# arclabs561/innr

Measured on NVIDIA B200. Metric: batch_knn_cosine_top10_queries_per_s, higher is better.
Workload: dtype f32

## Files before the change

### innr_b200/csrc/scan_f32.cu

```cuda
#include <algorithm>
#include <cmath>
#include <type_traits>

#include "common.cuh"
#include "kernels.cuh"
#include "pdx.cuh"

namespace innr {

namespace {

constexpr int SCAN_THREADS = 256;
constexpr int VPT = 4;
constexpr int TILE = SCAN_THREADS * VPT;
constexpr float NORM_EPS = 1e-9f;

struct PdxArgs {
  PdxView v;
  unsigned long long ld;
  unsigned n, d, ld4;
  unsigned n_tiles;
  unsigned index_base;
  const float* queries;
  int nq_valid;
// ... 726 lines not shown
    float ss = 0.0f;
    for (unsigned i = 0; i < d; ++i) ss = __fadd_rn(ss, __fmul_rn(query[i], query[i]));
    s_qn = __fsqrt_rn(ss);
  }
  __syncthreads();
  const unsigned j = blockIdx.x * blockDim.x + threadIdx.x;
  if (j >= m) return;
  const unsigned gid = cand[j];
  const unsigned i = gid - index_base;
  if (gid < index_base || i >= n) {
    out[j] = MODE == PDX_L2 ? __int_as_float(0x7FC00000) : __int_as_float(0xFFC00000);
    return;
  }
  float acc = 0.0f, ss = 0.0f;
  for (unsigned dd = 0; dd < d; ++dd) {
    const float x = pdx_load1(v, (size_t)dd * v.ld + i);
    accumulate<MODE == PDX_COSINE_FUSED ? PDX_DOT : MODE>(sq[dd], x, acc);
    if (MODE == PDX_COSINE_FUSED) ss = __fadd_rn(ss, __fmul_rn(x, x));
  }
  float sc = acc;
  if (MODE == PDX_COSINE_FUSED) {
    const float nrm = __fsqrt_rn(ss), qn = s_qn;
    sc = (!(qn < NORM_EPS) && nrm > NORM_EPS) ? __fdiv_rn(acc, __fmul_rn(qn, nrm)) : 0.0f;
  }
  out[j] = sc;
}
}

cudaError_t launch_subset_scores(const PdxView& v, int mode, const float* dev_query, const uint32_t* dev_cand, size_t m,
                                 float* dev_out, cudaStream_t s, LaunchCounter* launches) {
  if (m == 0) return cudaSuccess;
  const unsigned grid = (unsigned)((m + SCAN_THREADS - 1) / SCAN_THREADS);
  const size_t smem = ((v.d + 3) & ~(size_t)3) * sizeof(float);
  if (smem > 200 * 1024) return cudaErrorInvalidValue;
#define INNR_SUBSET(MODE)                                                                                           \
  {                                                                                                                 \
    auto kern = subset_scores_kernel<MODE>;                                                                         \
    if (smem > 48 * 1024) {                                                                                         \
      cudaError_t e = cudaFuncSetAttribute(kern, cudaFuncAttributeMaxDynamicSharedMemorySize, (int)smem);           \
      if (e != cudaSuccess) return e;                                                                               \
    }                                                                                                               \
    kern<<<grid, SCAN_THREADS, smem, s>>>(v, (unsigned)v.n, (unsigned)v.d, v.index_base, dev_query,                 \
                                          dev_cand, (unsigned)m, dev_out);                                          \
  }
  if (mode == PDX_DOT) INNR_SUBSET(PDX_DOT)
  else if (mode == PDX_L2) INNR_SUBSET(PDX_L2)
  else if (mode == PDX_COSINE_FUSED) INNR_SUBSET(PDX_COSINE_FUSED)
  else return cudaErrorInvalidValue;
#undef INNR_SUBSET
  ++*launches;
  return cudaGetLastError();
}

cudaError_t launch_topk_from_scores(const void* dev_scores, int kind, size_t n, uint32_t index_base, size_t k,
                                    uint64_t* dev_keys, Workspace& ws, cudaStream_t s, LaunchCounter* launches,
                                    const uint32_t* dev_ids, const uint32_t* dev_mask, unsigned seg_len, unsigned seg_stride) {
  unsigned grid = (unsigned)((n + SCAN_THREADS - 1) / SCAN_THREADS);
  unsigned cap = (unsigned)ws.num_sms * 4u;
  if (grid > cap) grid = cap;
  if (grid == 0) grid = 1;
  for (size_t done = 0; done < k; done += 128) {
    const int kr = (int)std::min<size_t>(128, k - done);
    const uint64_t* floor = done ? dev_keys + done - 1 : nullptr;
    uint64_t* out = dev_keys + done;
    const size_t smem = (size_t)(SCAN_THREADS / 32) * kr * sizeof(uint64_t);
#define INNR_TOPK_LAUNCH(R, KIND)                                                                                   \
  topk_scores_kernel<R, KIND><<<grid, SCAN_THREADS, smem, s>>>(dev_scores, (unsigned)n, index_base, dev_ids, dev_mask, seg_len, seg_stride, kr, floor, \
                                                               ws.partials, ws.group_partials, out, ws.tickets)
    if (kr <= 32) {
      if (kind == 0) INNR_TOPK_LAUNCH(1, 0); else if (kind == 1) INNR_TOPK_LAUNCH(1, 1);
      else if (kind == 2) INNR_TOPK_LAUNCH(1, 2); else if (kind == 3) INNR_TOPK_LAUNCH(1, 3); else INNR_TOPK_LAUNCH(1, 4);
    } else {
      if (kind == 0) INNR_TOPK_LAUNCH(4, 0); else if (kind == 1) INNR_TOPK_LAUNCH(4, 1);
      else if (kind == 2) INNR_TOPK_LAUNCH(4, 2); else if (kind == 3) INNR_TOPK_LAUNCH(4, 3); else INNR_TOPK_LAUNCH(4, 4);
    }
#undef INNR_TOPK_LAUNCH
    ++*launches;
    cudaError_t e = cudaGetLastError();
    if (e != cudaSuccess) return e;
  }
  return cudaSuccess;
}

namespace {
__global__ void decode_keys_kernel(const uint64_t* __restrict__ keys, size_t total, int descending, uint64_t* __restrict__ idx,
                                   float* __restrict__ score) {
  const size_t t = (size_t)blockIdx.x * blockDim.x + threadIdx.x;
  if (t >= total) return;
  const uint64_t key = keys[t];
  if (idx) idx[t] = key & 0xFFFFFFFFull;
  if (score) {
    uint32_t hi = (uint32_t)(key >> 32);
    if (descending) hi = ~hi;
    score[t] = __uint_as_float(order_bits_to_f32_bits(hi));
  }
}
}

cudaError_t launch_merge_keys_big(const uint64_t* dev_in, size_t n_lists, size_t nq, size_t k, int descending,
                                  uint64_t* dev_keys_out, uint64_t* dev_idx, float* dev_score, Workspace& ws, cudaStream_t s,
                                  LaunchCounter* launches) {
  for (size_t q = 0; q < nq; ++q) {
    cudaError_t e = launch_topk_from_scores(dev_in + q * k, 3, n_lists * k, 0, k, dev_keys_out + q * k, ws, s, launches, nullptr,
                                            nullptr, (unsigned)k, (unsigned)(nq * k));
    if (e != cudaSuccess) return e;
  }
  if (dev_idx || dev_score) {
    const size_t total = nq * k;
    decode_keys_kernel<<<(unsigned)((total + 255) / 256), 256, 0, s>>>(dev_keys_out, total, descending, dev_idx, dev_score);
    ++*launches;
  }
  return cudaGetLastError();
}

namespace {

struct AdaptArgs {
  PdxView v;
  unsigned long long ld;
  unsigned ld4;
  const float* query;
  unsigned d0, d1;
  float* dist;
  const uint32_t* mask_in;
  uint32_t* mask_out;
  const float* thr;
  uint32_t* ev;
  unsigned* pruned;
  int no_prune;
};

__global__ void __launch_bounds__(SCAN_THREADS) adaptive_epoch_kernel(const AdaptArgs a) {
  extern __shared__ __align__(16) unsigned char smem_raw[];
  float* sq = reinterpret_cast<float*>(smem_raw);
  const unsigned nd = a.d1 - a.d0;
  for (unsigned j = threadIdx.x; j < nd; j += blockDim.x) sq[j] = a.query[a.d0 + j];
  __syncthreads();
  const int lane = threadIdx.x & 31;
  const unsigned i0 = (blockIdx.x * SCAN_THREADS + threadIdx.x) * VPT;
  const bool in = i0 < a.ld4;
  unsigned nib = in ? (a.mask_in[i0 >> 5] >> (i0 & 31)) & 0xFu : 0u;
  unsigned n_dead = 0;
  if (nib) {
    float4 acc = *reinterpret_cast<const float4*>(a.dist + i0);
    const float T = a.thr[0];
    unsigned ex = 0, e0 = 0, e1 = 0, e2 = 0, e3 = 0;
    size_t p = (size_t)a.d0 * a.ld + i0;
    auto step = [&](const float4& v, unsigned j) {
      const float q = sq[j];
      float df;
      df = __fsub_rn(q, v.x); acc.x = __fadd_rn(acc.x, __fmul_rn(df, df));
      df = __fsub_rn(q, v.y); acc.y = __fadd_rn(acc.y, __fmul_rn(df, df));
      df = __fsub_rn(q, v.z); acc.z = __fadd_rn(acc.z, __fmul_rn(df, df));
      df = __fsub_rn(q, v.w); acc.w = __fadd_rn(acc.w, __fmul_rn(df, df));
      if (!(ex & 1u) && acc.x > T) { ex |= 1u; e0 = a.d0 + j; }
      if (!(ex & 2u) && acc.y > T) { ex |= 2u; e1 = a.d0 + j; }
      if (!(ex & 4u) && acc.z > T) { ex |= 4u; e2 = a.d0 + j; }
      if (!(ex & 8u) && acc.w > T) { ex |= 8u; e3 = a.d0 + j; }
    };
    constexpr int U = 8;
    unsigned j = 0;
    for (; j + U <= nd; j += U) {
      float4 v[U];
#pragma unroll
      for (int u = 0; u < U; ++u) v[u] = pdx_load4(a.v, p + (size_t)u * a.ld);
      p += (size_t)U * a.ld;
#pragma unroll
      for (int u = 0; u < U; ++u) step(v[u], j + u);
    }
    for (; j < nd; ++j) {
      const float4 v = pdx_load4(a.v, p);
      p += a.ld;
      step(v, j);
    }
    *reinterpret_cast<float4*>(a.dist + i0) = acc;
    if (!a.no_prune) {
      const unsigned dead = ex & nib;
      if (dead & 1u) a.ev[i0] = e0;
      if (dead & 2u) a.ev[i0 + 1] = e1;
      if (dead & 4u) a.ev[i0 + 2] = e2;
      if (dead & 8u) a.ev[i0 + 3] = e3;
      nib &= ~dead;
      n_dead = __popc(dead);
    }
  }
  unsigned w = nib << (4 * (lane & 7));
  w |= __shfl_xor_sync(FULL_MASK, w, 1);
  w |= __shfl_xor_sync(FULL_MASK, w, 2);
  w |= __shfl_xor_sync(FULL_MASK, w, 4);
  if (in && (lane & 7) == 0) a.mask_out[i0 >> 5] = w;
#pragma unroll
  for (int o = 16; o > 0; o >>= 1) n_dead += __shfl_xor_sync(FULL_MASK, n_dead, o);
  if (lane == 0 && n_dead) atomicAdd(a.pruned, n_dead);
}

__global__ void adaptive_threshold_kernel(const uint64_t* key, float scale, float* thr) {
  const float t = __fmul_rn(__uint_as_float(order_bits_to_f32_bits((uint32_t)(*key >> 32))), scale);
  thr[0] = t;
  thr[1] = __fmul_rn(t, 1.5f);
}

__global__ void __launch_bounds__(SCAN_THREADS) adaptive_mark_kernel(const float* __restrict__ dist, unsigned n, unsigned ld4,
                                                                    float ratio, const float* __restrict__ thr,
                                                                    uint32_t* __restrict__ mask_out, unsigned* pruned) {
  const int lane = threadIdx.x & 31;
  const unsigned i = blockIdx.x * SCAN_THREADS + threadIdx.x;
  const unsigned words32 = (ld4 + 31u) / 32u * 32u;
  bool alive = false, dead = false;
  if (i < n) {
    dead = __fmul_rn(dist[i], ratio) > thr[1];
    alive = !dead;
  }
  const unsigned w = __ballot_sync(FULL_MASK, alive);
  const unsigned nd = __popc(__ballot_sync(FULL_MASK, dead));
  if (lane == 0) {
    if (i < words32) mask_out[i >> 5] = w;
    if (nd) atomicAdd(pruned, nd);
  }
}

__global__ void __launch_bounds__(SCAN_THREADS) adaptive_event_keys_kernel(const uint32_t* __restrict__ before,
                                                                          const uint32_t* __restrict__ after,
                                                                          const uint32_t* __restrict__ ev, unsigned n,
                                                                          uint64_t* __restrict__ keys) {
  const unsigned i = blockIdx.x * SCAN_THREADS + threadIdx.x;
  if (i >= n) return;
  const bool event = ((before[i >> 5] & ~after[i >> 5]) >> (i & 31)) & 1u;
  keys[i] = event ? ~(((uint64_t)ev[i] << 32) | i) : KEY_SENTINEL;
}

__global__ void adaptive_revive_kernel(const uint64_t* __restrict__ keys, unsigned m, uint32_t* mask) {
  const unsigned t = blockIdx.x * blockDim.x + threadIdx.x;
  if (t >= m) return;
  const unsigned i = (unsigned)(~keys[t] & 0xFFFFFFFFull);
  atomicOr(mask + (i >> 5), 1u << (i & 31));
}

}

cudaError_t launch_adaptive_threshold(const uint64_t* dev_key, float scale, float* dev_thr, cudaStream_t s,
                                      LaunchCounter* launches) {
  adaptive_threshold_kernel<<<1, 1, 0, s>>>(dev_key, scale, dev_thr);
  ++*launches;
  return cudaGetLastError();
}

cudaError_t launch_adaptive_mark(const PdxView& v, const float* dev_dist, float ratio, const float* dev_thr,
                                 uint32_t* dev_mask_out, unsigned* dev_pruned, cudaStream_t s, LaunchCounter* launches) {
  const unsigned ld4 = (unsigned)std::min<size_t>(v.ld, (v.n + 3) / 4 * 4);
  const unsigned span = (ld4 + 31u) / 32u * 32u;
  adaptive_mark_kernel<<<(span + SCAN_THREADS - 1) / SCAN_THREADS, SCAN_THREADS, 0, s>>>(dev_dist, (unsigned)v.n, ld4, ratio,
                                                                                      dev_thr, dev_mask_out, dev_pruned);
  ++*launches;
  return cudaGetLastError();
}

cudaError_t launch_adaptive_epoch(const PdxView& v, const float* dev_query, size_t d0, size_t d1, float* dev_dist,
                                  const uint32_t* dev_mask_in, uint32_t* dev_mask_out, const float* dev_thr, uint32_t* dev_ev,
                                  unsigned* dev_pruned, int no_prune, cudaStream_t s, LaunchCounter* launches) {
  AdaptArgs a{};
  a.v = v;
  a.ld = v.ld;
  a.ld4 = (unsigned)std::min<size_t>(v.ld, (v.n + 3) / 4 * 4);
  a.query = dev_query;
  a.d0 = (unsigned)d0;
  a.d1 = (unsigned)d1;
  a.dist = dev_dist;
  a.mask_in = dev_mask_in;
  a.mask_out = dev_mask_out;
  a.thr = dev_thr;
  a.ev = dev_ev;
  a.pruned = dev_pruned;
  a.no_prune = no_prune;
  const unsigned span = (a.ld4 + 31u) / 32u * 32u;
  const unsigned grid = (span / VPT + SCAN_THREADS - 1) / SCAN_THREADS;
  adaptive_epoch_kernel<<<grid, SCAN_THREADS, (d1 - d0) * sizeof(float), s>>>(a);
  ++*launches;
  return cudaGetLastError();
}

cudaError_t launch_adaptive_event_keys(const uint32_t* dev_before, const uint32_t* dev_after, const uint32_t* dev_ev, size_t n,
                                       uint64_t* dev_keys, cudaStream_t s, LaunchCounter* launches) {
  adaptive_event_keys_kernel<<<(unsigned)((n + SCAN_THREADS - 1) / SCAN_THREADS), SCAN_THREADS, 0, s>>>(dev_before, dev_after,
                                                                                                     dev_ev, (unsigned)n, dev_keys);
  ++*launches;
  return cudaGetLastError();
}

cudaError_t launch_adaptive_revive(const uint64_t* dev_keys, size_t m, uint32_t* dev_mask, cudaStream_t s,
                                   LaunchCounter* launches) {
  if (m == 0) return cudaSuccess;
  adaptive_revive_kernel<<<(unsigned)((m + 255) / 256), 256, 0, s>>>(dev_keys, (unsigned)m, dev_mask);
  ++*launches;
  return cudaGetLastError();
}

cudaError_t launch_topk_from_distances(const float* dev_dist, size_t n, size_t k, uint64_t* dev_keys,
                                       Workspace& ws, cudaStream_t s, LaunchCounter* launches) {
  return launch_topk_from_scores(dev_dist, 0, n, 0, k, dev_keys, ws, s, launches, nullptr, nullptr, 1, 1);
}

namespace {

constexpr int SC_VPT = 16;
constexpr int SC_TILE = SCAN_THREADS * SC_VPT;
constexpr int SC_U = 8;
constexpr int RS_WARPS = 4;

struct ScreenArgs {
  PdxSketch sk;
  unsigned long long ld;
  unsigned n, d, ld16, n_tiles, index_base;
  int k;
  const float* query;
  const float* norms;
  float gamma, eta, nu;
  uint64_t* partials;
  uint64_t* group_partials;
  unsigned* tickets;
  uint64_t* tkeys;
  float* opt;
  float* pess;
  unsigned* ctl;
};

struct alignas(16) ScreenQuery {
  float qn_ref, qn_up;
  float qq_lo, qq_hi;
  float q128;
  float e1;
  float gq;
  float unscale;
  unsigned wmax[SCAN_THREADS / 32];
};

template <int MODE>
__device__ __forceinline__ void screen_bounds(float acc, float s, float r, float nv, const ScreenQuery& c,
                                              const ScreenArgs& a, float& lower, float& upper) {
  const float g = a.gamma;
  const float v_up = __fmul_ru(__fadd_ru(__fmul_ru(nv, 1.0f + 0x1p-23f), a.nu), __fadd_ru(1.0f, g));
  if (!(__fmul_ru(c.qn_up, v_up) <= 0x1p100f)) {
    lower = -INFINITY;
    upper = INFINITY;
    return;
  }
  const float m_lo = __fsub_rd(__fsub_rd(__fmul_rd(acc, c.unscale), c.q128), c.e1);
  const float m_hi = __fadd_ru(__fsub_ru(__fmul_ru(acc, c.unscale), c.q128), c.e1);
  const float qr = __fmul_ru(c.qn_up, r);
  const float x_lo = __fsub_rd(__fmul_rd(s, m_lo), qr);
  const float x_hi = __fadd_ru(__fmul_ru(s, m_hi), qr);
  if (MODE == PDX_L2) {
    const float n_lo = __fmul_rd(nv, 1.0f - 0x1p-23f);
    const float vv_lo = fmaxf(0.0f, __fmul_rd(__fsub_rd(__fmul_rd(n_lo, n_lo), a.eta), __fsub_rd(1.0f, g)));
    const float l_lo = fmaxf(0.0f, __fadd_rd(__fsub_rd(c.qq_lo, 2.0f * x_hi), vv_lo));
    const float l_hi = __fadd_ru(__fsub_ru(c.qq_hi, 2.0f * x_lo), __fmul_ru(v_up, v_up));
    lower = fmaxf(0.0f, __fsub_rd(__fmul_rd(l_lo, __fsub_rd(1.0f, g)), a.eta));
    upper = __fadd_ru(__fmul_ru(l_hi, __fadd_ru(1.0f, g)), a.eta);
    if (!(upper <= 3.0e38f)) { lower = -INFINITY; upper = INFINITY; }
    return;
  }
  const float e = __fmaf_ru(c.gq, v_up, a.eta);
  lower = __fsub_rd(x_lo, e);
  upper = __fadd_ru(x_hi, e);
  if (MODE == PDX_COSINE_FUSED) {
    if (!(nv > NORM_EPS)) {
      lower = upper = 0.0f;
      return;
    }
    const float p = __fmul_rn(c.qn_ref, nv);
    lower = __fdiv_rd(lower, p);
    upper = __fdiv_ru(upper, p);
  }
}

template <int MODE, int R>
__global__ void __launch_bounds__(SCAN_THREADS) pdx_screen_kernel(const ScreenArgs a) {
  extern __shared__ __align__(16) unsigned char smem_raw[];
  const unsigned d_pad = (a.d + 31u) / 32u * 32u;
  float* sq = reinterpret_cast<float*>(smem_raw);
  float* sqs = sq + d_pad;
  ScreenQuery* sc = reinterpret_cast<ScreenQuery*>(sqs + d_pad);
  uint64_t* smem_keys = reinterpret_cast<uint64_t*>(sc + 1);
  const int lane = threadIdx.x & 31;
  unsigned mb = 0;
  for (unsigned dd = threadIdx.x; dd < d_pad; dd += blockDim.x) {
    const float x = dd < a.d ? a.query[dd] : 0.0f;
    sq[dd] = x;
    mb = max(mb, __float_as_uint(x) & 0x7FFFFFFFu);
  }
  mb = __reduce_max_sync(FULL_MASK, mb);
  if (lane == 0) sc->wmax[threadIdx.x >> 5] = mb;
  __syncthreads();
#pragma unroll
  for (int w = 0; w < SCAN_THREADS / 32; ++w) mb = max(mb, sc->wmax[w]);
  if (!(mb >= 0x0D800000u && mb <= 0x71800000u)) {
    if (threadIdx.x == 0) a.ctl[1] = 1u;
    return;
  }
  const int p = 253 - (int)(mb >> 23);
  const float f1 = __uint_as_float((unsigned)(p / 2 + 127) << 23), f2 = __uint_as_float((unsigned)(p - p / 2 + 127) << 23);
  for (unsigned dd = threadIdx.x; dd < d_pad; dd += blockDim.x) sqs[dd] = __fmul_rn(__fmul_rn(sq[dd], f1), f2);
  __syncthreads();
  if (threadIdx.x == SCAN_THREADS - 1) {
    float ss = 0.0f, su = 0.0f, sl = 0.0f, qs = 0.0f, sa = 0.0f;
    for (unsigned dd = 0; dd < a.d; ++dd) {
      const float x = sq[dd];
      ss = __fadd_rn(ss, __fmul_rn(x, x));
      su = __fmaf_ru(x, x, su);
      sl = __fmaf_rd(x, x, sl);
      qs = __fadd_rn(qs, x);
      sa = __fadd_ru(sa, fabsf(x));
    }
    const float us = __uint_as_float((unsigned)(276 - p) << 23);
    sc->qn_ref = __fsqrt_rn(ss);
    sc->qn_up = __fsqrt_ru(su);
    sc->qq_lo = sl;
    sc->qq_hi = su;
    sc->q128 = 128.0f * qs;
    sc->e1 = __fadd_ru(__fmul_ru(a.gamma, __fmul_ru(383.0f, sa)), __fmul_ru(__uint_as_float(a.d), us));
    sc->gq = __fmul_ru(a.gamma, sc->qn_up);
    sc->unscale = us;
  }
  bool qn_visible = false;
  WarpList<R> lists[1];
  lists[0].init();
  uint64_t thr = KEY_SENTINEL;

  for (unsigned tile = blockIdx.x; tile < a.n_tiles; tile += gridDim.x) {
    const unsigned i0 = tile * SC_TILE + threadIdx.x * SC_VPT;
    const bool active = i0 < a.ld16;
    uint64_t acc[SC_VPT / 2];
#pragma unroll
    for (int j = 0; j < SC_VPT / 2; ++j) acc[j] = 0;
    auto step = [&](const uint4& w, float q) {
      const uint64_t q2 = pack2(q, q);
      const unsigned x[4] = {w.x, w.y, w.z, w.w};
#pragma unroll
      for (int t = 0; t < 4; ++t) {
        const float b0 = __uint_as_float(__byte_perm(x[t], 0u, 0x4440u)), b1 = __uint_as_float(__byte_perm(x[t], 0u, 0x4441u));
        const float b2 = __uint_as_float(__byte_perm(x[t], 0u, 0x4442u)), b3 = __uint_as_float(__byte_perm(x[t], 0u, 0x4443u));
        acc[2 * t] = fma2_rn(q2, pack2(b0, b1), acc[2 * t]);
        acc[2 * t + 1] = fma2_rn(q2, pack2(b2, b3), acc[2 * t + 1]);
      }
    };
    if (active) {
      const uint8_t* p = a.sk.codes + pdx_sketch_off(a.ld, 0, i0);
      const size_t next = pdx_sketch_off(a.ld, 1, 0);
      unsigned dd = 0;
      for (; dd + SC_U <= a.d; dd += SC_U) {
        uint4 w[SC_U];
#pragma unroll
        for (int u = 0; u < SC_U; ++u) w[u] = ldg_stream_u4(reinterpret_cast<const uint4*>(p + u * next));
        p += SC_U * next;
#pragma unroll
        for (int u = 0; u < SC_U; ++u) step(w[u], sqs[dd + u]);
      }
      for (; dd < a.d; ++dd, p += next) step(ldg_stream_u4(reinterpret_cast<const uint4*>(p)), sqs[dd]);
    }
    if (!qn_visible) {
      __syncthreads();
      qn_visible = true;
      const float qr = sc->qn_ref, qu = sc->qn_up;
      if (!(qu <= 0x1p100f) || (MODE == PDX_COSINE_FUSED && !(qr >= NORM_EPS))) {
        if (threadIdx.x == 0) a.ctl[1] = 1u;
        return;
      }
    }
#pragma unroll
    for (int h = 0; h < SC_VPT / 4; ++h) {
      const unsigned ih = i0 + 4 * h;
      float lo[4] = {0.0f, 0.0f, 0.0f, 0.0f}, up[4] = {0.0f, 0.0f, 0.0f, 0.0f};
      if (active) {
        const float4 s4 = *reinterpret_cast<const float4*>(a.sk.scale + ih);
        const float4 r4 = *reinterpret_cast<const float4*>(a.sk.resid + ih);
        const float4 n4 = *reinterpret_cast<const float4*>(a.norms + ih);
        const float s[4] = {s4.x, s4.y, s4.z, s4.w}, r[4] = {r4.x, r4.y, r4.z, r4.w}, nv[4] = {n4.x, n4.y, n4.z, n4.w};
        float x[4];
        unpack2(acc[2 * h], x[0], x[1]);
        unpack2(acc[2 * h + 1], x[2], x[3]);
#pragma unroll
        for (int j = 0; j < 4; ++j) screen_bounds<MODE>(x[j], s[j], r[j], nv[j], *sc, a, lo[j], up[j]);
        const float* ob = (MODE == PDX_L2) ? lo : up;
        *reinterpret_cast<float4*>(a.opt + ih) = make_float4(ob[0], ob[1], ob[2], ob[3]);
        if (a.pess) {
          const float* pb = (MODE == PDX_L2) ? up : lo;
          for (int j = 0; j < 4; ++j) a.pess[ih + j] = pb[j];
        }
      }
#pragma unroll
      for (int j = 0; j < 4; ++j) {
        const unsigned i = ih + j;
        const uint64_t key = (MODE == PDX_L2) ? make_key_asc(up[j], a.index_base + i) : make_key_desc(lo[j], a.index_base + i);
        lists[0].offer(key, active && i < a.n, thr, a.k, lane);
      }
    }
  }
  block_finish<R, 1>(lists, 1, a.k, smem_keys, a.partials, a.group_partials, a.tkeys, a.tickets);
}

__global__ void __launch_bounds__(SCAN_THREADS) screen_compact_kernel(const float* __restrict__ opt, unsigned n, int l2,
                                                                      const uint64_t* __restrict__ tkeys, int k,
                                                                      unsigned index_base, uint32_t* __restrict__ cand,
                                                                      unsigned* ctl) {
  if (ctl[1]) return;
  const uint64_t kth = tkeys[k - 1];
  float t;
  if (kth == KEY_SENTINEL) t = l2 ? INFINITY : -INFINITY;
  else t = __uint_as_float(order_bits_to_f32_bits(l2 ? (uint32_t)(kth >> 32) : ~(uint32_t)(kth >> 32)));
  const int lane = threadIdx.x & 31;
  const unsigned stride = gridDim.x * blockDim.x, n_round = (n + 31u) / 32u * 32u;
  for (unsigned i = blockIdx.x * blockDim.x + threadIdx.x; i < n_round; i += stride) {
    bool hit = false;
    if (i < n) {
      const float b = opt[i];
      hit = l2 ? !(b > t) : !(b < t);
    }
    const unsigned m = __ballot_sync(FULL_MASK, hit);
    if (!m) continue;
    unsigned base = 0;
    if (lane == 0) base = atomicAdd(&ctl[0], (unsigned)__popc(m));
    base = __shfl_sync(FULL_MASK, base, 0);
    const unsigned pos = base + __popc(m & ((1u << lane) - 1u));
    if (hit && pos < SCREEN_CAP) cand[pos] = index_base + i;
  }
}

template <int MODE>
__global__ void __launch_bounds__(RS_WARPS * 32) screen_rescore_kernel(const PdxView v, const float* __restrict__ query,
                                                                       const float* __restrict__ norms,
                                                                       const uint32_t* __restrict__ cand,
                                                                       unsigned* ctl, uint64_t* __restrict__ keys) {
  extern __shared__ __align__(16) unsigned char smem_raw[];
  const unsigned d = (unsigned)v.d, d_pad = (d + 3u) & ~3u;
  const int warp = threadIdx.x >> 5, lane = threadIdx.x & 31;
  float* sq = reinterpret_cast<float*>(smem_raw) + (size_t)2 * d_pad * warp;
  float* buf = sq + d_pad;
  const unsigned j = blockIdx.x * RS_WARPS + warp;
  const unsigned cnt = ctl[0], stop = ctl[1];
  if (j == 0 && lane == 0 && cnt > SCREEN_CAP) ctl[1] = 1u;
  if (stop || j >= min(cnt, (unsigned)SCREEN_CAP)) {
    if (lane == 0) keys[j] = KEY_SENTINEL;
    return;
  }
  for (unsigned dd = lane; dd < d; dd += 32) sq[dd] = query[dd];
  const unsigned gid = cand[j], i = gid - v.index_base;
  for (unsigned dd = lane; dd < d; dd += 32) buf[dd] = pdx_load1(v, (size_t)dd * v.ld + i);
  __syncwarp();
  if (lane != 0) return;
  float acc = 0.0f, qss = 0.0f;
  for (unsigned dd = 0; dd < d; ++dd) {
    const float q = sq[dd], x = buf[dd];
    accumulate<MODE == PDX_COSINE_FUSED ? PDX_DOT : MODE>(q, x, acc);
    if (MODE == PDX_COSINE_FUSED) qss = __fadd_rn(qss, __fmul_rn(q, q));
  }
  float sc = acc;
  if (MODE == PDX_COSINE_FUSED) {
    const float qn = __fsqrt_rn(qss), nrm = norms[i];
    sc = (!(qn < NORM_EPS) && nrm > NORM_EPS) ? __fdiv_rn(acc, __fmul_rn(qn, nrm)) : 0.0f;
  }
  keys[j] = MODE == PDX_L2 ? make_key_asc(sc, gid) : make_key_desc(sc, gid);
}

ScreenArgs screen_args(const PdxView& v, const float* dev_norms, const PdxSketch& sk, const float* dev_query, size_t k,
                       Workspace& ws) {
  ScreenArgs a{};
  a.sk = sk;
  a.ld = v.ld;
  a.n = (unsigned)v.n;
  a.d = (unsigned)v.d;
  a.ld16 = (unsigned)std::min<size_t>(v.ld, (v.n + 15) / 16 * 16);
  a.n_tiles = (unsigned)(((size_t)a.ld16 + SC_TILE - 1) / SC_TILE);
  a.index_base = v.index_base;
  a.k = (int)k;
  a.query = dev_query;
  a.norms = dev_norms;
  const double du = (double)(v.d + 2) * 0x1p-24;
  a.gamma = (float)(du / (1.0 - du)) * (1.0f + 0x1p-20f);
  a.eta = (float)((double)v.d * 0x1p-148) * (1.0f + 0x1p-20f) + 0x1p-149f;
  a.nu = (float)std::sqrt((double)v.d * 0x1p-149) * (1.0f + 0x1p-20f);
  a.partials = ws.partials;
  a.group_partials = ws.group_partials;
  a.tickets = ws.tickets;
  a.tkeys = ws.sc_keys + SCREEN_CAP;
  a.opt = ws.sc_bounds;
  a.ctl = ws.sc_ctl;
  return a;
}

template <int MODE, int R>
cudaError_t launch_screen(const ScreenArgs& a, int num_sms, cudaStream_t s) {
  auto kern = pdx_screen_kernel<MODE, R>;
  const size_t smem = (size_t)2 * ((a.d + 31u) / 32u * 32u) * sizeof(float) + sizeof(ScreenQuery) +
                      (size_t)(SCAN_THREADS / 32) * a.k * sizeof(uint64_t);
  static size_t smem_set_dev[16] = {};
  size_t& smem_set = smem_set_dev[current_device_slot()];
  if (smem > 48 * 1024 && smem > smem_set) {
    cudaError_t e = cudaFuncSetAttribute(kern, cudaFuncAttributeMaxDynamicSharedMemorySize, (int)smem);
    if (e != cudaSuccess) return e;
    smem_set = smem;
  }
  int occ = 0;
  cudaError_t e = cudaOccupancyMaxActiveBlocksPerMultiprocessor(&occ, kern, SCAN_THREADS, smem);
  if (e != cudaSuccess) return e;
  if (occ < 1) return cudaErrorInvalidConfiguration;
  kern<<<balanced_grid(a.n_tiles, (unsigned)occ * (unsigned)num_sms), SCAN_THREADS, smem, s>>>(a);
  return cudaGetLastError();
}

cudaError_t launch_screen_mode(int mode, const ScreenArgs& a, int num_sms, cudaStream_t s) {
  const bool big = a.k > 32;
  switch (mode) {
    case PDX_DOT: return big ? launch_screen<PDX_DOT, 4>(a, num_sms, s) : launch_screen<PDX_DOT, 1>(a, num_sms, s);
    case PDX_COSINE_FUSED:
      return big ? launch_screen<PDX_COSINE_FUSED, 4>(a, num_sms, s) : launch_screen<PDX_COSINE_FUSED, 1>(a, num_sms, s);
    case PDX_L2: return big ? launch_screen<PDX_L2, 4>(a, num_sms, s) : launch_screen<PDX_L2, 1>(a, num_sms, s);
  }
  return cudaErrorInvalidValue;
}

}

cudaError_t launch_pdx_knn_screened(const PdxView& v, int mode, const float* dev_norms, const PdxSketch& sk,
                                    const float* dev_query, size_t k, uint64_t* dev_keys, Workspace& ws, cudaStream_t s,
                                    LaunchCounter* launches) {
  if (!v.hi || !sk.codes || k == 0 || k > 128 || v.d == 0 || v.d > SCREEN_MAX_D || v.n < k || ws.sc_bounds_cap < v.ld)
    return cudaErrorInvalidValue;
  const ScreenArgs a = screen_args(v, dev_norms, sk, dev_query, k, ws);
  cudaError_t e = cudaMemsetAsync(ws.sc_ctl, 0, 2 * sizeof(unsigned), s);
  if (e != cudaSuccess) return e;
  if ((e = launch_screen_mode(mode, a, ws.num_sms, s)) != cudaSuccess) return e;
  screen_compact_kernel<<<(unsigned)std::min<size_t>((v.n + SCAN_THREADS - 1) / SCAN_THREADS, (size_t)ws.num_sms * 8), SCAN_THREADS, 0, s>>>(
      ws.sc_bounds, (unsigned)v.n, mode == PDX_L2, a.tkeys, (int)k, v.index_base, ws.sc_cand, ws.sc_ctl);
  const size_t rs_smem = (size_t)(2 * RS_WARPS) * ((v.d + 3) & ~(size_t)3) * sizeof(float);
#define INNR_RESCORE(MODE)                                                                                              \
  {                                                                                                                     \
    auto kern = screen_rescore_kernel<MODE>;                                                                            \
    if (rs_smem > 48 * 1024 && (e = cudaFuncSetAttribute(kern, cudaFuncAttributeMaxDynamicSharedMemorySize, (int)rs_smem)) != cudaSuccess) \
      return e;                                                                                                         \
    kern<<<(unsigned)(SCREEN_CAP / RS_WARPS), RS_WARPS * 32, rs_smem, s>>>(v, dev_query, dev_norms, ws.sc_cand, ws.sc_ctl, ws.sc_keys); \
  }
  if (mode == PDX_DOT) INNR_RESCORE(PDX_DOT)
  else if (mode == PDX_L2) INNR_RESCORE(PDX_L2)
  else INNR_RESCORE(PDX_COSINE_FUSED)
#undef INNR_RESCORE
  *launches += 3;
  if ((e = cudaGetLastError()) != cudaSuccess) return e;
  if ((e = launch_topk_from_scores(ws.sc_keys, 3, SCREEN_CAP, 0, k, dev_keys, ws, s, launches)) != cudaSuccess) return e;
  return launch_pdx_knn(v, mode, dev_query, 1, k, dev_keys, ws, s, launches, ws.sc_ctl + 1);
}

cudaError_t launch_pdx_screen_debug_bounds(const PdxView& v, int mode, const float* dev_norms, const PdxSketch& sk,
                                           const float* dev_query, float* host_lower, float* host_upper, Workspace& ws,
                                           cudaStream_t s, LaunchCounter* launches) {
  if (!v.hi || !sk.codes || v.n == 0 || v.d == 0 || v.d > SCREEN_MAX_D || 2 * v.ld > ws.sc_bounds_cap)
    return cudaErrorInvalidValue;
  ScreenArgs a = screen_args(v, dev_norms, sk, dev_query, 1, ws);
  a.pess = ws.sc_bounds + v.ld;
  cudaError_t e = cudaMemsetAsync(ws.sc_ctl, 0, 2 * sizeof(unsigned), s);
  if (e != cudaSuccess) return e;
  if ((e = launch_screen_mode(mode, a, ws.num_sms, s)) != cudaSuccess) return e;
  ++*launches;
  unsigned flag[2];
  if ((e = cudaMemcpyAsync(flag, ws.sc_ctl, sizeof(flag), cudaMemcpyDeviceToHost, s)) != cudaSuccess) return e;
  if ((e = cudaStreamSynchronize(s)) != cudaSuccess) return e;
  if (flag[1]) return cudaErrorNotSupported;
  float* lower = mode == PDX_L2 ? a.opt : a.pess;
  float* upper = mode == PDX_L2 ? a.pess : a.opt;
  if ((e = cudaMemcpyAsync(host_lower, lower, v.n * sizeof(float), cudaMemcpyDeviceToHost, s)) != cudaSuccess) return e;
  if ((e = cudaMemcpyAsync(host_upper, upper, v.n * sizeof(float), cudaMemcpyDeviceToHost, s)) != cudaSuccess) return e;
  return cudaStreamSynchronize(s);
}

}
```

Before: 781.8.

## Split screen kernel dimension loop across warps with smem reduction and adaptive VPT

Reworks the sketch screening kernel so each warp handles a slice of the dimension range for a 32*VPT row tile, then reduces the partial dot products through double-buffered shared memory before computing bounds. A launcher picks VPT 16, 8 or 4 by how well the grid fills the SMs. It also adds min-CTA launch bounds, double-buffered code loads, cached occupancy queries and a few spare CTAs. The aim is better SM fill and latency hiding on smaller corpora, paid for with a __syncthreads per tile, more shared memory and a cross-warp reduction.

```diff
diff --git a/innr_b200/csrc/dev/screen_ab.py b/innr_b200/csrc/dev/screen_ab.py
--- /dev/null
+++ b/innr_b200/csrc/dev/screen_ab.py
@@ -0,0 +1,125 @@
+import argparse
+import ctypes as C
+import json
+import os
+import subprocess
+import sys
+
+import numpy as np
+import torch
+
+sys.path.insert(0, ".")
+from innr_b200 import _lib as L, synth
+
+ap = argparse.ArgumentParser()
+ap.add_argument("--lib", action="append", default=[], help="NAME=PATH of a libinnr_cuda.so build")
+ap.add_argument("--sizes", default="10000000,5000000,2500000,1250000")
+ap.add_argument("--rounds", type=int, default=5)
+ap.add_argument("--calls", type=int, default=40)
+ap.add_argument("--out", default=None)
+args = ap.parse_args()
+libs = dict(s.split("=", 1) for s in args.lib) or {"tree": L.SO_PATH}
+D, K, NQ = 768, 10, 16
+
+
+def smi():
+    q = "name,power.limit,clocks.max.sm,clocks.sm,temperature.gpu"
+    return subprocess.run(["nvidia-smi", f"--query-gpu={q}", "--format=csv,noheader"], capture_output=True,
+                          text=True).stdout.strip().splitlines()[0]
+
+
+def load(path):
+    lib = C.CDLL(os.path.abspath(path))
+    for name, argtypes in L.SIGNATURES.items():
+        getattr(lib, name).restype = C.c_int
+        getattr(lib, name).argtypes = argtypes
+    lib.innr_cuda_last_error.restype = C.c_char_p
+    return lib
+
+
+def check(lib, rc):
+    if rc:
+        raise RuntimeError(lib.innr_cuda_last_error().decode())
+
+
+torch.cuda.init()
+handles = {}
+for name, path in libs.items():
+    handles[name] = load(path)
+    check(handles[name], handles[name].innr_cuda_init(0))
+    check(handles[name], handles[name].innr_cuda_set_option(b"f32_split_min_rows", 0.0))
+q = torch.from_numpy(synth.ghash_f32(synth.SALT_QUERY, 0, NQ * D).reshape(NQ, D)).cuda()
+stream = torch.cuda.current_stream()
+report = {"gpu_before": smi(), "libs": libs, "sizes": {}}
+print("gpu:", report["gpu_before"])
+
+
+def call(name, corpus, i, out):
+    lib = handles[name]
+    check(lib, lib.innr_cuda_batch_knn_keys_dev(corpus, L.METRIC_COSINE, C.c_void_p(q[i % NQ].data_ptr()), 1, K,
+                                                C.c_void_p(out.data_ptr()), C.c_void_p(stream.cuda_stream)))
+
+
+def time_calls(name, corpus, out):
+    e0, e1 = torch.cuda.Event(enable_timing=True), torch.cuda.Event(enable_timing=True)
+    e0.record()
+    for i in range(args.calls):
+        call(name, corpus, i, out)
+    e1.record()
+    torch.cuda.synchronize()
+    return e0.elapsed_time(e1) / args.calls
+
+
+def screen_ms(name, corpus, out, calls=20):
+    from torch.profiler import ProfilerActivity, profile
+    with profile(activities=[ProfilerActivity.CUDA]) as prof:
+        for i in range(calls):
+            call(name, corpus, i, out)
+        torch.cuda.synchronize()
+    t = 0.0
+    for ev in prof.key_averages():
+        if ev.device_type.name == "CUDA" and "pdx_screen_kernel" in ev.key:
+            t += (getattr(ev, "device_time_total", None) or getattr(ev, "cuda_time_total", 0)) / calls / 1000.0
+    return t
+
+
+for n in [int(s) for s in args.sizes.split(",")]:
+    corpora = {}
+    for name, lib in handles.items():
+        h = C.c_void_p()
+        check(lib, lib.innr_cuda_generate_f32_pdx(0, synth.SALT_CORPUS, 0, n, D, 0, C.byref(h)))
+        corpora[name] = h
+    keys = {}
+    for name in handles:
+        keys[name] = torch.empty(NQ * K, dtype=torch.int64, device="cuda")
+        for i in range(NQ):
+            call(name, corpora[name], i, keys[name][i * K:(i + 1) * K])
+    torch.cuda.synchronize()
+    first = next(iter(keys.values()))
+    equal = all(bool(torch.equal(first, v)) for v in keys.values())
+    one = torch.empty(K, dtype=torch.int64, device="cuda")
+    call_ms = {name: [] for name in handles}
+    scr_ms = {name: [] for name in handles}
+    for r in range(args.rounds):
+        for name in handles:
+            call_ms[name].append(time_calls(name, corpora[name], one))
+    for r in range(3):
+        for name in handles:
+            scr_ms[name].append(screen_ms(name, corpora[name], one))
+    screen_bytes = n * D + n * 16
+    res = {"n": n, "keys_equal_across_builds_16_queries": equal, "screen_bytes": screen_bytes, "builds": {}}
+    for name in handles:
+        cm, sm = float(np.median(call_ms[name])), float(np.median(scr_ms[name]))
+        res["builds"][name] = {"call_ms": call_ms[name], "call_ms_median": cm, "screen_ms": scr_ms[name],
+                               "screen_ms_median": sm, "screen_tb_per_s": screen_bytes / (sm / 1e3) / 1e12}
+    report["sizes"][str(n)] = res
+    print(json.dumps(res))
+    for name, lib in handles.items():
+        check(lib, lib.innr_cuda_free(corpora[name]))
+    torch.cuda.synchronize()
+report["gpu_after"] = smi()
+print("gpu:", report["gpu_after"])
+if args.out:
+    os.makedirs(args.out, exist_ok=True)
+    with open(os.path.join(args.out, "screen_ab.json"), "w") as f:
+        json.dump(report, f, indent=1)
diff --git a/innr_b200/csrc/scan_f32.cu b/innr_b200/csrc/scan_f32.cu
--- a/innr_b200/csrc/scan_f32.cu
+++ b/innr_b200/csrc/scan_f32.cu
@@ -1052,10 +1052,12 @@
 
 namespace {
 
-constexpr int SC_VPT = 16;
-constexpr int SC_TILE = SCAN_THREADS * SC_VPT;
-constexpr int SC_U = 8;
+constexpr int SC_WARPS = SCAN_THREADS / 32;
+constexpr int SC_U = 4;
+template <int R>
+constexpr int sc_min_ctas() { return R == 1 ? 3 : 2; }
 constexpr int RS_WARPS = 4;
+constexpr unsigned SC_SPARE_CTAS = 8;
 
 struct ScreenArgs {
   PdxSketch sk;
@@ -1081,7 +1083,7 @@
   float e1;
   float gq;
   float unscale;
-  unsigned wmax[SCAN_THREADS / 32];
+  unsigned wmax[SC_WARPS];
 };
 
 template <int MODE>
@@ -1123,15 +1125,32 @@
   }
 }
 
-template <int MODE, int R>
-__global__ void __launch_bounds__(SCAN_THREADS) pdx_screen_kernel(const ScreenArgs a) {
+template <int VPT>
+__device__ __forceinline__ void ldg_codes(const uint8_t* p, unsigned (&x)[VPT / 4]) {
+  if constexpr (VPT == 16) {
+    const uint4 w = ldg_stream_u4(reinterpret_cast<const uint4*>(p));
+    x[0] = w.x, x[1] = w.y, x[2] = w.z, x[3] = w.w;
+  } else if constexpr (VPT == 8) {
+    asm volatile("ld.global.nc.L1::no_allocate.v2.u32 {%0, %1}, [%2];" : "=r"(x[0]), "=r"(x[1]) : "l"(p));
+  } else {
+    asm volatile("ld.global.nc.L1::no_allocate.u32 %0, [%1];" : "=r"(x[0]) : "l"(p));
+  }
+}
+
+template <int MODE, int R, int VPT>
+__global__ void __launch_bounds__(SCAN_THREADS, sc_min_ctas<R>()) pdx_screen_kernel(const ScreenArgs a) {
+  constexpr int W = VPT / 4;
+  constexpr int ROWS = 32 * VPT;
+  constexpr int EPW = ROWS / SC_WARPS;
+  constexpr int EPL = EPW >= 32 ? EPW / 32 : 1;
   extern __shared__ __align__(16) unsigned char smem_raw[];
   const unsigned d_pad = (a.d + 31u) / 32u * 32u;
   float* sq = reinterpret_cast<float*>(smem_raw);
   float* sqs = sq + d_pad;
   ScreenQuery* sc = reinterpret_cast<ScreenQuery*>(sqs + d_pad);
   uint64_t* smem_keys = reinterpret_cast<uint64_t*>(sc + 1);
-  const int lane = threadIdx.x & 31;
+  float* part = reinterpret_cast<float*>(smem_keys + (size_t)SC_WARPS * a.k);
+  const int lane = threadIdx.x & 31, warp = threadIdx.x >> 5;
   unsigned mb = 0;
   for (unsigned dd = threadIdx.x; dd < d_pad; dd += blockDim.x) {
     const float x = dd < a.d ? a.query[dd] : 0.0f;
@@ -1139,10 +1158,10 @@
     mb = max(mb, __float_as_uint(x) & 0x7FFFFFFFu);
   }
   mb = __reduce_max_sync(FULL_MASK, mb);
-  if (lane == 0) sc->wmax[threadIdx.x >> 5] = mb;
+  if (lane == 0) sc->wmax[warp] = mb;
   __syncthreads();
 #pragma unroll
-  for (int w = 0; w < SCAN_THREADS / 32; ++w) mb = max(mb, sc->wmax[w]);
+  for (int w = 0; w < SC_WARPS; ++w) mb = max(mb, sc->wmax[w]);
   if (!(mb >= 0x0D800000u && mb <= 0x71800000u)) {
     if (threadIdx.x == 0) a.ctl[1] = 1u;
     return;
@@ -1171,78 +1190,111 @@
     sc->gq = __fmul_ru(a.gamma, sc->qn_up);
     sc->unscale = us;
   }
-  bool qn_visible = false;
   WarpList<R> lists[1];
   lists[0].init();
   uint64_t thr = KEY_SENTINEL;
-
-  for (unsigned tile = blockIdx.x; tile < a.n_tiles; tile += gridDim.x) {
-    const unsigned i0 = tile * SC_TILE + threadIdx.x * SC_VPT;
-    const bool active = i0 < a.ld16;
-    uint64_t acc[SC_VPT / 2];
-#pragma unroll
-    for (int j = 0; j < SC_VPT / 2; ++j) acc[j] = 0;
-    auto step = [&](const uint4& w, float q) {
+  const unsigned d0 = (unsigned)warp * a.d / SC_WARPS, d1 = (unsigned)(warp + 1) * a.d / SC_WARPS;
+  const unsigned nb = (d1 - d0) / SC_U;
+  const unsigned next = (unsigned)pdx_sketch_off(a.ld, 1, 0);
+  const bool e_lane = lane * EPL < EPW;
+
+  unsigned it = 0;
+  for (unsigned tile = blockIdx.x; tile < a.n_tiles; tile += gridDim.x, ++it) {
+    const unsigned t0 = tile * ROWS, i0 = t0 + lane * VPT;
+    const unsigned r0 = warp * EPW + lane * EPL, e0 = t0 + r0;
+    const bool e_act = e_lane && e0 < a.ld16;
+    float s[EPL], r[EPL], nv[EPL];
+    if (e_act) {
+      if constexpr (EPL == 2) {
+        const float2 s2 = *reinterpret_cast<const float2*>(a.sk.scale + e0);
+        const float2 r2 = *reinterpret_cast<const float2*>(a.sk.resid + e0);
+        const float2 n2 = *reinterpret_cast<const float2*>(a.norms + e0);
+        s[0] = s2.x, s[1] = s2.y, r[0] = r2.x, r[1] = r2.y, nv[0] = n2.x, nv[1] = n2.y;
+      } else {
+        s[0] = a.sk.scale[e0], r[0] = a.sk.resid[e0], nv[0] = a.norms[e0];
+      }
+    }
+    uint64_t acc[VPT / 2];
+#pragma unroll
+    for (int j = 0; j < VPT / 2; ++j) acc[j] = 0;
+    auto step = [&](const unsigned (&x)[W], float q) {
       const uint64_t q2 = pack2(q, q);
-      const unsigned x[4] = {w.x, w.y, w.z, w.w};
-#pragma unroll
-      for (int t = 0; t < 4; ++t) {
+#pragma unroll
+      for (int t = 0; t < W; ++t) {
         const float b0 = __uint_as_float(__byte_perm(x[t], 0u, 0x4440u)), b1 = __uint_as_float(__byte_perm(x[t], 0u, 0x4441u));
         const float b2 = __uint_as_float(__byte_perm(x[t], 0u, 0x4442u)), b3 = __uint_as_float(__byte_perm(x[t], 0u, 0x4443u));
         acc[2 * t] = fma2_rn(q2, pack2(b0, b1), acc[2 * t]);
         acc[2 * t + 1] = fma2_rn(q2, pack2(b2, b3), acc[2 * t + 1]);
       }
     };
-    if (active) {
-      const uint8_t* p = a.sk.codes + pdx_sketch_off(a.ld, 0, i0);
-      const size_t next = pdx_sketch_off(a.ld, 1, 0);
-      unsigned dd = 0;
-      for (; dd + SC_U <= a.d; dd += SC_U) {
-        uint4 w[SC_U];
-#pragma unroll
-        for (int u = 0; u < SC_U; ++u) w[u] = ldg_stream_u4(reinterpret_cast<const uint4*>(p + u * next));
-        p += SC_U * next;
-#pragma unroll
-        for (int u = 0; u < SC_U; ++u) step(w[u], sqs[dd + u]);
-      }
-      for (; dd < a.d; ++dd, p += next) step(ldg_stream_u4(reinterpret_cast<const uint4*>(p)), sqs[dd]);
-    }
-    if (!qn_visible) {
-      __syncthreads();
-      qn_visible = true;
+    if (i0 < a.ld16) {
+      const uint8_t* p = a.sk.codes + pdx_sketch_off(a.ld, d0, i0);
+      unsigned x0[SC_U][W], x1[SC_U][W];
+      auto load = [&](unsigned (&x)[SC_U][W]) {
+#pragma unroll
+        for (int u = 0; u < SC_U; ++u) ldg_codes<VPT>(p + (size_t)u * next, x[u]);
+        p += (size_t)SC_U * next;
+      };
+      auto sum = [&](const unsigned (&x)[SC_U][W], unsigned dd) {
+#pragma unroll
+        for (int u = 0; u < SC_U; ++u) step(x[u], sqs[dd + u]);
+      };
+      if (nb) load(x0);
+      unsigned b = 0;
+      for (; b + 2 <= nb; b += 2) {
+        load(x1);
+        sum(x0, d0 + b * SC_U);
+        if (b + 2 < nb) load(x0);
+        sum(x1, d0 + (b + 1) * SC_U);
+      }
+      if (b < nb) sum(x0, d0 + b * SC_U);
+      for (unsigned dd = d0 + nb * SC_U; dd < d1; ++dd, p += next) {
+        unsigned x[W];
+        ldg_codes<VPT>(p, x);
+        step(x, sqs[dd]);
+      }
+    }
+    float* pb = part + (size_t)(it & 1u) * (SC_WARPS * ROWS);
+#pragma unroll
+    for (int j = 0; j < VPT / 4; ++j) {
+      float4 v;
+      unpack2(acc[2 * j], v.x, v.y);
+      unpack2(acc[2 * j + 1], v.z, v.w);
+      *reinterpret_cast<float4*>(pb + warp * ROWS + lane * VPT + 4 * j) = v;
+    }
+    __syncthreads();
+    if (it == 0) {
       const float qr = sc->qn_ref, qu = sc->qn_up;
       if (!(qu <= 0x1p100f) || (MODE == PDX_COSINE_FUSED && !(qr >= NORM_EPS))) {
         if (threadIdx.x == 0) a.ctl[1] = 1u;
         return;
       }
     }
-#pragma unroll
-    for (int h = 0; h < SC_VPT / 4; ++h) {
-      const unsigned ih = i0 + 4 * h;
-      float lo[4] = {0.0f, 0.0f, 0.0f, 0.0f}, up[4] = {0.0f, 0.0f, 0.0f, 0.0f};
-      if (active) {
-        const float4 s4 = *reinterpret_cast<const float4*>(a.sk.scale + ih);
-        const float4 r4 = *reinterpret_cast<const float4*>(a.sk.resid + ih);
-        const float4 n4 = *reinterpret_cast<const float4*>(a.norms + ih);
-        const float s[4] = {s4.x, s4.y, s4.z, s4.w}, r[4] = {r4.x, r4.y, r4.z, r4.w}, nv[4] = {n4.x, n4.y, n4.z, n4.w};
-        float x[4];
-        unpack2(acc[2 * h], x[0], x[1]);
-        unpack2(acc[2 * h + 1], x[2], x[3]);
-#pragma unroll
-        for (int j = 0; j < 4; ++j) screen_bounds<MODE>(x[j], s[j], r[j], nv[j], *sc, a, lo[j], up[j]);
-        const float* ob = (MODE == PDX_L2) ? lo : up;
-        *reinterpret_cast<float4*>(a.opt + ih) = make_float4(ob[0], ob[1], ob[2], ob[3]);
-        if (a.pess) {
-          const float* pb = (MODE == PDX_L2) ? up : lo;
-          for (int j = 0; j < 4; ++j) a.pess[ih + j] = pb[j];
-        }
-      }
-#pragma unroll
-      for (int j = 0; j < 4; ++j) {
-        const unsigned i = ih + j;
-        const uint64_t key = (MODE == PDX_L2) ? make_key_asc(up[j], a.index_base + i) : make_key_desc(lo[j], a.index_base + i);
-        lists[0].offer(key, active && i < a.n, thr, a.k, lane);
-      }
+    float lo[EPL], up[EPL];
+#pragma unroll
+    for (int e = 0; e < EPL; ++e) {
+      lo[e] = up[e] = 0.0f;
+      if (e_act) {
+        float x = pb[r0 + e];
+#pragma unroll
+        for (int w = 1; w < SC_WARPS; ++w) x = __fadd_rn(x, pb[w * ROWS + r0 + e]);
+        screen_bounds<MODE>(x, s[e], r[e], nv[e], *sc, a, lo[e], up[e]);
+      }
+    }
+    if (e_act) {
+      const float* ob = (MODE == PDX_L2) ? lo : up;
+      if constexpr (EPL == 2) *reinterpret_cast<float2*>(a.opt + e0) = make_float2(ob[0], ob[1]);
+      else a.opt[e0] = ob[0];
+      if (a.pess) {
+        const float* pv = (MODE == PDX_L2) ? up : lo;
+        for (int e = 0; e < EPL; ++e) a.pess[e0 + e] = pv[e];
+      }
+    }
+#pragma unroll
+    for (int e = 0; e < EPL; ++e) {
+      const unsigned i = e0 + e;
+      const uint64_t key = (MODE == PDX_L2) ? make_key_asc(up[e], a.index_base + i) : make_key_desc(lo[e], a.index_base + i);
+      lists[0].offer(key, e_act && i < a.n, thr, a.k, lane);
     }
   }
   block_finish<R, 1>(lists, 1, a.k, smem_keys, a.partials, a.group_partials, a.tkeys, a.tickets);
@@ -1319,7 +1371,6 @@
   a.n = (unsigned)v.n;
   a.d = (unsigned)v.d;
   a.ld16 = (unsigned)std::min<size_t>(v.ld, (v.n + 15) / 16 * 16);
-  a.n_tiles = (unsigned)(((size_t)a.ld16 + SC_TILE - 1) / SC_TILE);
   a.index_base = v.index_base;
   a.k = (int)k;
   a.query = dev_query;
@@ -1337,23 +1388,60 @@
   return a;
 }
 
+struct ScreenFit {
+  size_t smem;
+  unsigned tiles, grid, slots;
+};
+
+template <int MODE, int R, int VPT>
+cudaError_t screen_fit(const ScreenArgs& a, int num_sms, ScreenFit& f) {
+  auto kern = pdx_screen_kernel<MODE, R, VPT>;
+  f.smem = (size_t)2 * ((a.d + 31u) / 32u * 32u) * sizeof(float) + sizeof(ScreenQuery) +
+           (size_t)SC_WARPS * a.k * sizeof(uint64_t) + (size_t)2 * SC_WARPS * 32 * VPT * sizeof(float);
+  const int dev = current_device_slot();
+  static size_t smem_set_dev[16] = {}, occ_smem_dev[16] = {};
+  static int occ_dev[16] = {};
+  if (f.smem > 48 * 1024 && f.smem > smem_set_dev[dev]) {
+    cudaError_t e = cudaFuncSetAttribute(kern, cudaFuncAttributeMaxDynamicSharedMemorySize, (int)f.smem);
+    if (e != cudaSuccess) return e;
+    smem_set_dev[dev] = f.smem;
+  }
+  if (occ_smem_dev[dev] != f.smem) {
+    cudaError_t e = cudaOccupancyMaxActiveBlocksPerMultiprocessor(&occ_dev[dev], kern, SCAN_THREADS, f.smem);
+    if (e != cudaSuccess) return e;
+    occ_smem_dev[dev] = f.smem;
+  }
+  if (occ_dev[dev] < 1) return cudaErrorInvalidConfiguration;
+  f.tiles = (a.ld16 + 32u * VPT - 1) / (32u * VPT);
+  f.slots = (unsigned)occ_dev[dev] * (unsigned)num_sms;
+  f.grid = balanced_grid(f.tiles, f.slots > SC_SPARE_CTAS ? f.slots - SC_SPARE_CTAS : f.slots);
+  return cudaSuccess;
+}
+
+template <int MODE, int R, int VPT>
+void screen_launch(ScreenArgs a, const ScreenFit& f, cudaStream_t s) {
+  a.n_tiles = f.tiles;
+  pdx_screen_kernel<MODE, R, VPT><<<f.grid, SCAN_THREADS, f.smem, s>>>(a);
+}
+
 template <int MODE, int R>
 cudaError_t launch_screen(const ScreenArgs& a, int num_sms, cudaStream_t s) {
-  auto kern = pdx_screen_kernel<MODE, R>;
-  const size_t smem = (size_t)2 * ((a.d + 31u) / 32u * 32u) * sizeof(float) + sizeof(ScreenQuery) +
-                      (size_t)(SCAN_THREADS / 32) * a.k * sizeof(uint64_t);
-  static size_t smem_set_dev[16] = {};
-  size_t& smem_set = smem_set_dev[current_device_slot()];
-  if (smem > 48 * 1024 && smem > smem_set) {
-    cudaError_t e = cudaFuncSetAttribute(kern, cudaFuncAttributeMaxDynamicSharedMemorySize, (int)smem);
-    if (e != cudaSuccess) return e;
-    smem_set = smem;
-  }
-  int occ = 0;
-  cudaError_t e = cudaOccupancyMaxActiveBlocksPerMultiprocessor(&occ, kern, SCAN_THREADS, smem);
-  if (e != cudaSuccess) return e;
-  if (occ < 1) return cudaErrorInvalidConfiguration;
-  kern<<<balanced_grid(a.n_tiles, (unsigned)occ * (unsigned)num_sms), SCAN_THREADS, smem, s>>>(a);
+  ScreenFit f[3];
+  cudaError_t e;
+  if ((e = screen_fit<MODE, R, 16>(a, num_sms, f[0])) != cudaSuccess) return e;
+  if ((e = screen_fit<MODE, R, 8>(a, num_sms, f[1])) != cudaSuccess) return e;
+  if ((e = screen_fit<MODE, R, 4>(a, num_sms, f[2])) != cudaSuccess) return e;
+  int pick = 0;
+  for (int i = 0; i < 3; ++i) {
+    if ((size_t)f[i].grid * 20 >= (size_t)f[i].slots * 19) {
+      pick = i;
+      break;
+    }
+    if ((size_t)f[i].grid * f[pick].slots > (size_t)f[pick].grid * f[i].slots) pick = i;
+  }
+  if (pick == 0) screen_launch<MODE, R, 16>(a, f[0], s);
+  else if (pick == 1) screen_launch<MODE, R, 8>(a, f[1], s);
+  else screen_launch<MODE, R, 4>(a, f[2], s);
   return cudaGetLastError();
 }
 
```

Result: faster. 818.1 (median of 6 runs) (+4.6%).
